# Nextomics/NextPolish2

Measured on AMD Instinct MI355X. Metric: polished reference Mbp/s (whole node) at 30x HiFi + k21/k31; FASTA identical to oracle, higher is better.
Workload: dtype u8

## Files before the change

### nextpolish2_amd/csrc/np2_ctx.hpp

```cpp
#pragma once
#include "../../include/np2.h"
#include "np2_abi.hpp"
#include "np2_common.hpp"
#include "np2_kernels.hpp"
#include "np2_hostcpu.hpp"

#include <algorithm>
#include <atomic>
#include <chrono>
#include <cstdio>
#include <cstdlib>
#include <cstring>
#include <map>
#include <memory>
#include <exception>
#include <mutex>
#include <stdexcept>
#include <string>
#include <vector>

namespace np2h {

using namespace np2;

// ... 488 lines not shown
    uint32_t chunk_epoch = 0;
    DevBuf<uint32_t> tile_cur, tile_n, tile_scan, tile_scanb, tile_nn, tile_nr, tile_noff, tile_roff;
    uint32_t tile_cap = TILE_CAP;
    uint32_t bucket_cap = 0;
    DevBuf<uint2> nrec;
    DevBuf<uint8_t> votebuf;
    DevBuf<uint32_t> band, band_n, band_off, row_cnt;
    DevBuf<int64_t> run_gain, tile_gain;
    DevBuf<uint8_t> out_snap;
    DevBuf<uint8_t> run_flag;
    uint32_t deep_min = 65536;
    DevBuf<uint32_t> lq_list, hbits;
    DevBuf<uint16_t> tile_pidx;
    bool pidx_valid = false;
    DevBuf<ReadInfo> rinfo;
    DevBuf<uint32_t> lqc, lqoff;
    DevBuf<uint8_t> pflag;
    DevBuf<uint32_t> dp_list;
    DevBuf<uint16_t> pf_slots;
    DevBuf<uint32_t> pf_bad, pf_bad2;
    DevBuf<uint64_t> pf_prof;
    bool front_fused = false;
    struct Hooks {
        bool front_unfused = false, pf_prof = false, edge_sort = false;
        bool test_misspeculate = false, shard_spec_log = false, phase_profile = false, exact_grow = false, no_speculate = false;
        bool has_grow_guess = false, rech_general = false, rech_log = false;
        uint32_t grow_guess = 0;
        uint32_t rech_cap_list = 0xFFFFFFFFu, rech_cap_jobs = 0xFFFFFFFFu, rech_cap_blob = 0xFFFFFFFFu;
        bool has_pf_cap = false, has_pf_cap_big = false, has_pf_halo = false, has_pf_cov_max = false;
        uint32_t pf_cap = 0, pf_cap_big = 0, pf_halo = 0, pf_cov_max = 0;
        void read() {
            auto on = [](const char *n) { return getenv(n) != nullptr; };
            auto u32 = [](const char *n, bool &has, uint32_t &v) {
                if (const char *e = getenv(n)) has = true, v = (uint32_t)atol(e);
            };
            front_unfused = on("NP2_FRONT_UNFUSED"), pf_prof = on("NP2_PF_PROF"), edge_sort = on("NP2_EDGE_SORT");
            test_misspeculate = on("NP2_TEST_MISSPECULATE");
            shard_spec_log = on("NP2_SHARD_SPEC_LOG"), phase_profile = on("NP2_PHASE_PROFILE"), exact_grow = on("NP2_EXACT_GROW");
            no_speculate = on("NP2_NO_SPECULATE");
            rech_general = on("NP2_RECH_GENERAL");
            rech_log = on("NP2_RECH_LOG");
            if (const char *e = getenv("NP2_TEST_RECH_CAP")) {
                char *end = nullptr;
                rech_cap_list = (uint32_t)strtoul(e, &end, 10);
                if (end && *end == ',') rech_cap_jobs = (uint32_t)strtoul(end + 1, &end, 10);
                if (end && *end == ',') rech_cap_blob = (uint32_t)strtoul(end + 1, &end, 10);
            }
            u32("NP2_TEST_GROW_GUESS", has_grow_guess, grow_guess);
            u32("NP2_PF_CAP", has_pf_cap, pf_cap), u32("NP2_PF_CAP_BIG", has_pf_cap_big, pf_cap_big);
            u32("NP2_PF_HALO", has_pf_halo, pf_halo), u32("NP2_PF_COV_MAX", has_pf_cov_max, pf_cov_max);
        }
    } hooks;
    bool pf_big = getenv("NP2_PF_BIG") != nullptr;
    uint32_t front_redos = 0;
    DevBuf<uint16_t> kscore_saved;
    DevBuf<uint8_t> sstr;
    DevBuf<uint64_t> soff;
    DevBuf<uint16_t> sscore;
};


namespace np2h {


enum Scal { S_ERR = 0, S_NNODES, S_NRUNS, S_BEST, S_PATHBEGIN, S_NRAW, S_NREG, S_DUP, S_LAST0, S_LAST1, S_GAIN0,
            S_GAIN1, S_DEEP, S_NDPLIST, S_NRECH, S_NGROUPS, S_NLONG, S_NLQ, S_PF, S_M0, S_M1, S_M2, S_M3, S_NC, S_SB, S_GROW,
            S_NBAD, S_PFOUT, S_PFGAIN0, S_PFGAIN1, S_PFEND0, S_PFEND1, S_NBAD2, S_NOKEY, S_COUNT = 34 };
static_assert(S_M1 % 2 == 0 && S_LAST0 % 2 == 0 && S_GAIN0 % 2 == 0 && S_PFGAIN0 % 2 == 0 && S_PFEND0 % 2 == 0,
              "64-bit device counters live in these slot pairs");

static constexpr int NP2_MAX_YAK = 15;
static constexpr uint32_t SCAL_TOTAL = 96;
static_assert(S_COUNT + 2 * (NP2_MAX_YAK + 2) <= SCAL_TOTAL && S_COUNT < 64, "round counters behind the posted block; the mailbox holds 64 words");
static constexpr uint32_t S_RL = S_COUNT + 2 * (NP2_MAX_YAK + 2);
static_assert(S_RL + 2 + np2::RL_STATE_WORDS <= SCAL_TOTAL, "the region lists' counters fit behind the round counters");

inline double thread_cpu_ms() {
    timespec ts;
    clock_gettime(CLOCK_THREAD_CPUTIME_ID, &ts);
    return ts.tv_sec * 1e3 + ts.tv_nsec * 1e-6;
}
struct WallTimer {
    np2_ctx *cx;
    const char *name;
    double t0, c0 = 0;
    WallTimer(np2_ctx *c, const char *n);
    ~WallTimer();
};

struct EventTimer {
// ... 245 lines not shown
```

### nextpolish2_amd/csrc/np2_host.cpp

```cpp
#include "../../include/np2.h"
#include "np2_common.hpp"
#include "np2_kernels.hpp"
#include "np2_ctx.hpp"
#include "np2_phase_host.hpp"

#include <algorithm>
#include <atomic>
#include <thread>
#include <chrono>
#include <cstdio>
#include <cstdlib>
#include <cstring>
#include <map>
#include <mutex>
#include <stdexcept>
#include <string>
#include <unordered_map>
#include <unordered_set>
#include <future>
#include <functional>
#include <vector>

using namespace np2;

// ... 100 lines not shown
    (void)cx;
    if (e & 4u) throw Np2Error(NP2_E_REFPANIC, "reference would panic: seq2 order is equal to 0");
    if (e & 8u) throw Np2Error(NP2_E_REFPANIC, "reference would panic: index out of bounds: lqseq.seqs[max1_p]");
    if (e & 16u) throw Np2Error(NP2_E_REFPANIC, "reference would panic: the first lqseq is not ref.");
    if (e & 32u) throw Np2Error(NP2_E_REFPANIC, "reference would panic: lqseq.seqs[0] after retain_sort_seqs");
    if (e & 64u) throw Np2Error(NP2_E_REFPANIC, "reference would panic: consensus index out of bounds in reupdate");
    if (e & 128u) throw Np2Error(NP2_E_NOMEM, "cartesian product of chained LQ regions is too large");
    if (e & LB_ERR) throw Np2Error(NP2_E_DEVICE, "device-wide scan timed out waiting for a predecessor block");
    if (e & (GROW_ERR | RECH_CAP_ERR)) throw GrowRetry((e & GROW_ERR) != 0, (e & RECH_CAP_ERR) != 0);
    if (e & LQ_LIST_ERR) throw Np2Error(NP2_E_DEVICE, "internal: more low-quality bases than their list was sized for");
}

struct VoteData {
    uint32_t R = 0;
    bool any = false;
    std::vector<uint64_t> pair_key;
    std::vector<uint32_t> pair_cnt;
    const uint64_t *view_key = nullptr;
    const uint32_t *view_cnt = nullptr;
    uint64_t view_n = 0;
    const uint32_t *off = nullptr;
    const phase::Graph::Edge *edges = nullptr;
    uint32_t n_nokey = 0;
    std::vector<uint32_t> off_own;
    std::vector<phase::Graph::Edge> edges_own;
    bool rows() const { return off != nullptr; }
    const uint64_t *keys() const { return view_key ? view_key : pair_key.data(); }
    const uint32_t *cnts() const { return view_key ? view_cnt : pair_cnt.data(); }
    uint64_t n_pairs() const { return view_key ? view_n : (uint64_t)pair_key.size(); }
    void own() {
        if (rows() && off_own.empty()) {
            off_own.assign(off, off + R + 1);
            edges_own.assign(edges, edges + off[R]);
            off = off_own.data(), edges = edges_own.data();
        }
        if (!view_key) return;
        pair_key.assign(view_key, view_key + view_n);
        pair_cnt.assign(view_cnt, view_cnt + view_n);
        view_key = nullptr, view_cnt = nullptr, view_n = 0;
    }
    std::vector<uint32_t> first_key;
    std::vector<int32_t> ref_w;
    std::vector<uint8_t> ref_seen, bad;
    const uint8_t *d_bad = nullptr;
    bool key_added = false;
};
// ... 50 lines not shown
        cx->ecount.ensure(n_reg + 2);
        cx->eoff.ensure(std::max<size_t>(n_reg + 2, (size_t)c->L + 2));
        const size_t RP = ((size_t)R + 63) & ~(size_t)63;
        const size_t band_words = (size_t)R * EDGE_BAND;
        const size_t b_v = RP * 10, b_off = (((size_t)R + 2) * 4 + 15) & ~(size_t)15;
        uint8_t *vbuf;
        uint32_t *row_off;
        if (wide) {
            cx->votebuf.ensure(b_v);
            cx->band_off.ensure((size_t)R + 2);
            vbuf = cx->votebuf.p, row_off = cx->band_off.p;
        } else {
            cx->votepack.ensure(b_v + b_off + band_words * 2 * sizeof(phase::Graph::Edge) + 64);
            vbuf = cx->votepack.p, row_off = (uint32_t *)(cx->votepack.p + b_v);
        }
        uint32_t *v_first = (uint32_t *)vbuf;
        int32_t *v_refw = (int32_t *)(vbuf + RP * 4);
        uint8_t *v_seen = vbuf + RP * 8, *v_bad = vbuf + RP * 9;
        op_fill(cx, v_first, 0xFF, RP * 4);
        op_fill(cx, v_refw, 0, RP * 6);
        launch_vote_phase(s, rt, asref, use_all, cx->lq_start.p, own_lo, own_hi, cx->reg_lable.p, cx->grp.p, cx->ecount.p,
                          v_refw, v_seen, v_bad, v_first, cx->scal.p + S_ERR);
        exclusive_total_n(cx, cx->ecount.p, cx->eoff.p, n_reg);
        launch_vote_counts(s, v_first, v_bad, R, cx->scal.p + S_M1);
        cx->band.ensure(band_words + 4);
        cx->band_n.ensure((size_t)R + 2);
        op_fill(cx, cx->scal.p + S_M3, 0, 4);
        launch_edges_row(s, rt, cx->grp.p, cx->ecount.p, cx->pj.p, cx->pcount.p, cx->alive.p, R, cx->band.p, cx->band_n.p,
                         cx->scal.p + S_M3);
        if (wide) {
            exclusive_total_n(cx, cx->band_n.p, row_off, R);
            cx->ekey.ensure(band_words + 2);
            cx->eval.ensure(band_words + 2);
            launch_band_emit(s, cx->band.p, R, row_off, cx->ekey.p, cx->eval.p, cx->scal.p + S_NRAW, key_add);
        } else {
            cx->row_cnt.ensure((size_t)R + 2);
            launch_vote_rows_count(s, cx->band.p, cx->band_n.p, v_bad, use_all, R, cx->row_cnt.p, cx->scal.p + S_NOKEY);
            exclusive_total_n(cx, cx->row_cnt.p, row_off, R);
            launch_vote_rows_emit(s, cx->band.p, cx->band_n.p, v_bad, use_all, v_first, R, row_off, cx->votepack.p + b_v + b_off,
                                  cx->scal.p + S_NRAW, cx->scal.p + S_NOKEY);
        }
    }
    const size_t RP = ((size_t)R + 63) & ~(size_t)63;
    const size_t b_v = RP * 10, b_off = (((size_t)R + 2) * 4 + 15) & ~(size_t)15;
    auto per_read = [&](const uint8_t *vb) {
        vd.first_key.assign((const uint32_t *)vb, (const uint32_t *)vb + R);
        vd.ref_w.assign((const int32_t *)(vb + RP * 4), (const int32_t *)(vb + RP * 4) + R);
        vd.ref_seen.assign(vb + RP * 8, vb + RP * 8 + R);
        vd.bad.assign(vb + RP * 9, vb + RP * 9 + R);
    };
    bool far = false, have_per_read = false;
    {
        std::vector<uint32_t> sc;
        uint8_t *pin = nullptr;
        const size_t EB = sizeof(phase::Graph::Edge);
        static_assert(sizeof(phase::Graph::Edge) == 8 && alignof(phase::Graph::Edge) <= 8, "an edge is {u32 neighbour, f32 weight}");
        const uint32_t likely = (uint32_t)std::min<size_t>((size_t)R * EDGE_BAND * 2, std::max<size_t>((size_t)R * 128, 1u << 15));
        if (wide) {
            sc = fetch_scal(cx, cx->scal.p + S_M0, cx->eoff.p + n_reg);
        } else {
            pin = (uint8_t *)cx->pin_d2h.ensure(b_v + b_off + (size_t)likely * EB + 64);
            const uint32_t seq = ++cx->mbox_seq;
            launch_post(cx->stream, cx->scal.p, S_COUNT, cx->mbox_dev, seq, cx->scal.p + S_M0, cx->eoff.p + n_reg, nullptr, nullptr,
                        nullptr, nullptr, nullptr, nullptr, nullptr, nullptr);
            op_d2h(cx, pin, cx->votepack.p, b_v + b_off);
            launch_copy_counted(cx->stream, (uint32_t *)(pin + b_v + b_off), (const uint32_t *)(cx->votepack.p + b_v + b_off),
                                (const uint32_t *)(cx->votepack.p + b_v) + R, likely * (uint32_t)(EB / 4), (uint32_t)(EB / 4));
            op_sync(cx);
            if (__atomic_load_n(&cx->mbox_host[0], __ATOMIC_ACQUIRE) != seq)
                throw Np2Error(NP2_E_DEVICE, "mailbox not posted after a synchronisation");
            sc.assign(cx->mbox_host + 1, cx->mbox_host + 1 + S_COUNT);
        }
        check_region_err(cx, sc[S_ERR]);
        pc.resolve(sc);
        NE = sc[S_M0];
        if (!cx->trace && sc[S_M1] == 0 && sc[S_M2] == 0) {
            if (NE) throw Np2Error(NP2_E_DEVICE, "internal: pair edges without voting reads");
            return;
        }
        NU = sc[S_NRAW];
        far = sc[S_M3] != 0 || cx->hooks.edge_sort;
        if (!wide) cx->timing.host.push_back({far ? "vote_sort" : "vote_rows", 1.0f});
        if (!wide) {
            per_read(pin);
            have_per_read = true;
            vd.d_bad = cx->votepack.p + RP * 9;
            if (!far) {
                if (NU > likely) {
                    pin = (uint8_t *)cx->pin_d2h.ensure(b_v + b_off + (size_t)NU * EB + 64);
                    op_d2h(cx, pin, cx->votepack.p, b_v + b_off + (size_t)NU * EB);
                    op_sync(cx);
                }
                vd.off = (const uint32_t *)(pin + b_v), vd.edges = (const phase::Graph::Edge *)(pin + b_v + b_off);
                vd.n_nokey = sc[S_NOKEY];
                if (vd.off[R] != NU) throw Np2Error(NP2_E_DEVICE, "internal: vote rows and edge count disagree");
            }
        }
    }
    vd.any = true;
    if (NE && far) {
        {
            EventTimer t(cx, "vote_phase");
            cx->ekey.ensure(NE + 2);
            cx->ekey_s.ensure(NE + 2);
            cx->eval.ensure(NE + 2);
// ... 29 lines not shown
            op_copy_d2d(cx, cx->votepack2.p + b_key, cx->eval.p, (size_t)NU * 4);
            if (b_pr) op_copy_d2d(cx, cx->votepack2.p + b_key + b_w, cx->votebuf.p, b_pr);
            op_d2h(cx, pin, cx->votepack2.p, b_key + b_w + b_pr);
        } else {
            op_d2h(cx, pin, cx->ekey.p, (size_t)NU * 8);
            op_d2h(cx, pin + b_key, cx->eval.p, (size_t)NU * 4);
            if (b_pr) op_d2h(cx, pin + b_key + b_w, cx->votebuf.p, b_pr);
        }
        op_sync(cx);
        vd.view_key = (const uint64_t *)pin, vd.view_cnt = (const uint32_t *)(pin + b_key), vd.view_n = NU;
        vd.key_added = wide && !far;
        if (b_pr) {
            per_read(pin + b_key + b_w);
            if (wide) vd.d_bad = cx->votebuf.p + RP * 9;
        }
    }
    if (cx->trace) {
        vd.own();
        trace_put(cx, pass, "hete.lable", d2h(cx, cx->reg_lable.p, n_reg));
        trace_put(cx, pass, "hete.kscore", d2h(cx, cx->kscore.p, pc.NC));
    }
}

std::vector<uint32_t> vote_decide(np2_ctx *cx, const VoteData &vd, bool use_all, int pass = -1) {
    if (!vd.any) return {};
    const uint32_t R = vd.R;
    const uint64_t NU = vd.rows() ? 0 : vd.n_pairs();
    const uint32_t *const pair_cnt = vd.rows() ? nullptr : vd.cnts();
    const double t_host0 = now_ms();
    std::vector<std::pair<uint32_t, uint32_t>> keys;
    for (uint32_t r = 0; r < R; ++r)
        if (vd.first_key[r] != 0xFFFFFFFFu) keys.emplace_back(vd.first_key[r], r);
    if (keys.size() < 4096) {
        std::sort(keys.begin(), keys.end());
    } else {
        std::vector<std::pair<uint32_t, uint32_t>> tmp(keys.size());
        std::vector<uint32_t> cnt(65537);
        for (int pass = 0; pass < 2; ++pass) {
            const int sh = 16 * pass;
            std::fill(cnt.begin(), cnt.end(), 0u);
            for (const auto &k : keys) ++cnt[((k.first >> sh) & 0xFFFFu) + 1];
            for (size_t i = 0; i < 65536; ++i) cnt[i + 1] += cnt[i];
            for (const auto &k : keys) tmp[cnt[(k.first >> sh) & 0xFFFFu]++] = k;
            keys.swap(tmp);
        }
    }
    const bool prof = getenv("NP2_PHASE_PROFILE") != nullptr;
    double t_mark = t_host0;
    auto mark = [&](const char *what) {
// ... 915 lines not shown
            if (cx->trace) trace_cns(cx, (int)r.pass, "cns_rech" + std::to_string(y), fetch_cns_dev(cx, cur));
        }
        fetch_result(cx, cur.pos, cur.base, cur.M_p, cur.M_cap, result, guessed ? r.M + r.grow_prev : r.M + pc.grow);
    } catch (const GrowRetry &g) {
        if ((g.grow && !guessed) || (g.rech_cap && !by_list)) throw;
        result.release();
        op_fill(cx, cx->scal.p + S_ERR, 0, 4);
        op_fill(cx, cx->scal.p + S_COUNT, 0, (size_t)(SCAL_TOTAL - S_COUNT) * 4);
        if (g.rech_cap) cx->timing.host.push_back({"rech_redo", 1.0f});
        r.reuse = false;
        run_final_pass(r, result, exact_grow || g.grow, rech_general || g.rech_cap);
    }
}

void polish_impl(np2_ctx *cx, np2_contig *c, const np2_opts_t *o, ResultOut &result) {
    PolishRun r;
    r.cx = cx, r.c = c, r.o = *o;
    run_begin(r);
    const bool no_spec = cx->hooks.no_speculate;
    const bool use_all = o->use_all_reads != 0;
    struct Decision {
        std::vector<uint32_t> losers;
        double ms = 0;
    };
    struct Pending {
        std::future<Decision> fut;
        std::shared_ptr<VoteData> vd;
        size_t n_bad = 0;
        bool active = false;
    } pend;
    auto settle = [&]() -> bool {
        if (!pend.active) return true;
        pend.active = false;
        Decision d = pend.fut.get();
        cx->timing.host.push_back({"wall_louvain", (float)d.ms});
        std::vector<uint32_t> extra;
        for (uint32_t id : d.losers) {
            REFPANIC_IF(id >= c->R, "index out of bounds: alignseqs[id]");
            if (!pend.vd->bad[id]) extra.push_back(id);
        }
        if (extra.empty() && d.losers.size() == pend.n_bad && !cx->hooks.test_misspeculate) return true;
        if (!extra.empty()) {
            cx->kill_ids.ensure(extra.size() + 1);
            h2d_staged(cx, cx->kill_ids.p, extra.data(), extra.size() * 4);
            launch_kill_reads(cx->stream, cx->kill_ids.p, (uint32_t)extra.size(), cx->alive.p);
        }
        r.reuse = false;
        r.front_issued = false;
        return false;
    };
    const std::function<void()> settle_then_redo = [&]() {
        if (!settle()) run_pass_front(r);
    };
    while (!r.final_pass()) {
        auto vd = std::make_shared<VoteData>();
        run_vote_pass(r, *vd, &settle_then_redo);
        size_t n_bad = 0;
        if (vd->any && vd->d_bad && !use_all && !cx->trace && !no_spec)
            for (uint8_t b : vd->bad) n_bad += b;
        if (n_bad == 0) {
            run_apply_losers(r, vote_decide(cx, *vd, use_all, (int)r.pass));
            continue;
        }
        launch_kill_flagged(cx->stream, vd->d_bad, c->R, cx->alive.p);
        ++r.pass;
        r.reuse = false;
        if (cx->hooks.pf_prof) vd->own();
        pass_front_issue(cx, c, r.T, (int)r.pass);
        r.front_issued = true;
        op_submit(cx);
        pend.vd = vd;
        pend.n_bad = n_bad;
        pend.active = true;
        auto decide = [vd, use_all]() {
            Decision d;
            const double t0 = now_ms();
            d.losers = vote_decide(nullptr, *vd, use_all);
            d.ms = now_ms() - t0;
            return d;
        };
        if (tl_recorder() == nullptr) {
            vd->own();
            pend.fut = std::async(std::launch::async, decide);
        } else {
            std::promise<Decision> p;
            pend.fut = p.get_future();
            try {
                p.set_value(decide());
            } catch (...) {
                p.set_exception(std::current_exception());
            }
            (void)settle();
        }
    }
    for (;;) {
        run_final_pass(r, result);
        if (settle()) break;
        result.release();
    }
}
// ... 811 lines not shown
            while (i < mk.size() && j < nx) {
                if (mk[i] < xk[j]) {
                    tk.push_back(mk[i]), tc.push_back(mc[i]), ++i;
                } else if (xk[j] < mk[i]) {
                    tk.push_back(xk[j]), tc.push_back(xc[j]), ++j;
                } else {
                    const uint32_t same = (mc[i] & 0xFFFFu) + (xc[j] & 0xFFFFu), neg = (mc[i] >> 16) + (xc[j] >> 16);
                    if (same > 0xFFFFu || neg > 0xFFFFu) return NP2_E_UNSUPPORTED;
                    tk.push_back(mk[i]), tc.push_back(same | (neg << 16)), ++i, ++j;
                }
            }
            tk.insert(tk.end(), mk.begin() + (long)i, mk.end());
            tc.insert(tc.end(), mc.begin() + (long)i, mc.end());
            tk.insert(tk.end(), xk + j, xk + nx);
            tc.insert(tc.end(), xc + j, xc + nx);
            mk.swap(tk), mc.swap(tc);
        }
        if (!vd.view_key) {
            vd.pair_key.swap(mk);
            vd.pair_cnt.swap(mc);
        }
        for (uint32_t r = 0; r < n_reads_total; ++r)
            if (votes_any[r]) vd.first_key[r] = 0xFFFFFFFEu - first_pos[r];
        if (getenv("NP2_VOTE_COMPACT")) {
            if (!vote_rows_from_pairs(vd, opts->use_all_reads != 0)) return NP2_E_UNSUPPORTED;
        }
        std::vector<uint32_t> ls = vote_decide(nullptr, vd, opts->use_all_reads != 0);
        *n_losers = (uint32_t)ls.size();
        for (size_t i = 0; i < ls.size(); ++i) losers[i] = ls[i];
        return NP2_OK;
    });
}

int np2_shard_apply(np2_shard_run_t *h, const uint32_t *losers, uint32_t n) {
    ShardRun *sr = (ShardRun *)h;
    if (!sr || (n && !losers) || (sr->run.final_pass() && !sr->spec)) return NP2_E_ARG;
    np2_ctx *cx = sr->run.cx;
    return abi_guard([&] {
        std::vector<uint32_t> local;
        const np2_shard_plan_t &pl = sr->plan;
        for (uint32_t i = 0; i < n; ++i) {
            if (losers[i] == 0) throw Np2Error(NP2_E_REFPANIC, "reference would panic: the contig itself was voted out");
            if (losers[i] >= pl.read_lo && losers[i] < pl.read_hi) local.push_back(losers[i] - pl.read_lo + 1);
        }
        if (sr->spec) {
            sr->spec = false;
            std::vector<uint32_t> extra, spared;
            size_t n_flagged = 0;
// ... 156 lines not shown
```

### nextpolish2_amd/csrc/np2_kernels.hpp

```cpp
#pragma once
#include <cstddef>
#include <cstdint>
#include <hip/hip_runtime.h>
#include "../../include/np2.h"
#include "np2_lookback.hpp"
#include "np2_launch.hpp"

namespace np2 {

static constexpr uint32_t TILE_SHIFT = 10;
static constexpr uint32_t TILE = 1u << TILE_SHIFT;
static constexpr uint32_t TILE_CAP = 4096;

static constexpr uint32_t DENSE_COLS = 4096;
struct ChunkDesc {
    uint64_t nib_off;
    uint64_t ckbase;
    uint32_t read, ts;
    uint32_t c0, ncols;
    uint32_t first_chunk;
    uint32_t aln_t_e, nck;
    uint32_t pad0;
    uint32_t pad[4];
};
// ... 238 lines not shown

struct RegionTables {
    const uint32_t *cand_off;
    const uint32_t *order;
    uint16_t *kscore;
    const uint32_t *seq_off;
    const uint8_t *seq;
    uint32_t n_reg;
};
struct RechPtrs {
    const void *groups;
    const uint32_t *job_off;
    const uint32_t *rech;
    const uint32_t *cand_off;
    const uint32_t *keep_list;
    const uint32_t *seq_off;
    const uint8_t *seq;
    const uint8_t *cns_base;
    uint32_t n_groups;
};
void launch_vote_phase(hipStream_t s, const RegionTables &rt, bool asref, bool use_all, const uint32_t *lq_start,
                       uint32_t own_lo, uint32_t own_hi, uint8_t *reg_lable, uint8_t *grp, uint32_t *ecount, int32_t *ref_w,
                       uint8_t *ref_seen, uint8_t *bad, uint32_t *first_reg, uint32_t *err);
void launch_vote_counts(hipStream_t s, const uint32_t *first_reg, const uint8_t *bad, uint32_t R, uint32_t *out);
void launch_edges_write(hipStream_t s, const RegionTables &rt, const uint8_t *reg_lable, const uint8_t *grp,
                        const uint32_t *ecount, const uint32_t *eoff, uint64_t *ekey, uint32_t *eval);
static constexpr uint32_t EDGE_BAND = 256;
void launch_edges_row(hipStream_t s, const RegionTables &rt, const uint8_t *grp, const uint32_t *ecount, const uint32_t *pj,
                      const uint32_t *pcount, const uint8_t *alive, uint32_t R, uint32_t *band, uint32_t *row_n, uint32_t *ovf);
void launch_band_emit(hipStream_t s, const uint32_t *band, uint32_t R, const uint32_t *row_off, uint64_t *ukey, uint32_t *uw,
                      uint32_t *n_out, uint64_t key_add = 0);
void launch_vote_rows_count(hipStream_t s, const uint32_t *band, const uint32_t *row_n, const uint8_t *bad, bool use_all, uint32_t R,
                            uint32_t *cnt, uint32_t *nokey);
void launch_vote_rows_emit(hipStream_t s, const uint32_t *band, const uint32_t *row_n, const uint8_t *bad, bool use_all,
                           const uint32_t *first_reg, uint32_t R, const uint32_t *off, void *edges, uint32_t *n_out, uint32_t *nokey);
void launch_edge_reduce(hipStream_t s, const uint64_t *ekey, const uint32_t *eval, uint32_t n, uint32_t *flag, uint32_t *wout);
void launch_edge_compact(hipStream_t s, const uint64_t *ekey, const uint32_t *flag, const uint32_t *idx, const uint32_t *wout,
                         uint32_t n, uint64_t *ukey, uint32_t *uw, uint32_t *n_out);
void launch_seed(hipStream_t s, const RegionTables &rt, int32_t max_indel_len, uint8_t *reg_lable, uint32_t *seed_cand,
                 uint32_t *keep_n, uint32_t *keep_list, uint16_t *keep_ks, uint32_t *err, uint32_t *rl_list = nullptr,
                 uint32_t *rl_cnt = nullptr, uint32_t rl_cap = 0);
uint32_t region_lb_blocks(uint32_t n_reg);
void launch_splice_find(hipStream_t s, const uint32_t *cns_pos, const uint32_t *M_p, const uint32_t *lq_start,
                        const uint32_t *lq_end, const uint8_t *reg_lable, uint8_t lable, uint32_t n_reg, uint32_t *idx_s,
                        uint32_t *idx_e, uint32_t *stuck);
void launch_splice_plan(hipStream_t s, const Lookback &lb, const uint8_t *reg_lable, uint8_t lable, uint32_t n_reg,
                        const uint32_t *stuck, const uint32_t *idx_s, const uint32_t *idx_e, const uint32_t *seed_cand,
                        const uint32_t *seq_off, uint32_t *ap_g, uint32_t *ap_s, uint32_t *ap_e, int32_t *ap_delta,
                        int32_t *ap_shift_incl, uint32_t *n_ap, const uint32_t *M_in, uint32_t *M_out, uint32_t out_cap , uint32_t *err);
void launch_splice_write(hipStream_t s, const uint32_t *in_pos, const uint8_t *in_base, const uint32_t *M_p, uint32_t M_cap,
                         const uint32_t *ap_g, const uint32_t *ap_s, const uint32_t *ap_e, const int32_t *ap_delta,
                         const int32_t *ap_shift_incl, const uint32_t *n_ap, uint32_t max_ap, const uint32_t *lq_start,
                         const uint32_t *seed_cand, const uint32_t *seq_off, const uint8_t *seq, uint32_t *out_pos,
                         uint8_t *out_base);
void launch_shard_bounds(hipStream_t s, const uint32_t *cns_pos, const uint32_t *M_p, const uint32_t *t, uint32_t *out);
void launch_rech_list(hipStream_t s, const Lookback &lb, const uint8_t *reg_lable, uint32_t n_reg, uint32_t *rech,
                      uint32_t *n_rech, unsigned long long *blob_bound, uint32_t *err);
void launch_rech_groups(hipStream_t s, const Lookback &lb, const uint32_t *rech, const uint32_t *n_rech_p, uint32_t max_rech,
// ... 71 lines not shown
```

### nextpolish2_amd/csrc/np2_regions.hip

```cpp
#include "np2_common.hpp"
#include "np2_kernels.hpp"
#include "np2_blockscan.hpp"
#include "np2_lookback.hpp"

namespace np2 {

static constexpr uint8_t LB_TEMP = 0x01, LB_SUCC = 0x80, LB_HETE = 0x40, LB_RECH = 0x20;

__device__ __forceinline__ uint32_t min_support(uint32_t n) { return n >= 9 ? 3u : (n >= 6 ? 2u : 1u); }

struct SubWave {
    uint32_t base;
    bool half;
    __device__ __forceinline__ uint64_t ballot(bool p) const {
        const uint64_t b = __ballot(p);
        return half ? (b >> base) & 0xFFFFFFFFull : b;
    }
    template <class T> __device__ __forceinline__ T shfl(T v, uint32_t j) const { return __shfl(v, (int)(base + j)); }
};

struct WaveStats {
    uint64_t eqmask;
    uint32_t stat;
    uint32_t c;
// ... 221 lines not shown
        gi = grp[c0 + lane];
        v = rt.kscore[c0 + lane] > 0;
    }
    uint64_t V = __ballot(v);
    if ((V & 1ull) && __shfl(order, 0) == 0) V &= ~1ull;
    const bool mine = (V >> lane) & 1ull;
    const uint32_t cnt = mine ? __builtin_popcountll(lane == 63 ? 0ull : (V >> (lane + 1))) : 0u;
    uint32_t inc = cnt;
    for (int o = 1; o < 64; o <<= 1) {
        const uint32_t t = __shfl_up(inc, o);
        if (lane >= (uint32_t)o) inc += t;
    }
    uint32_t o = eoff[g] + inc - cnt;
    for (uint32_t j = 1; j < n; ++j) {
        const uint32_t oj = __shfl(order, j), gj = __shfl(gi, j);
        if (mine && j > lane && ((V >> j) & 1ull)) {
            ekey[o] = ((uint64_t)order << 32) | oj;
            eval[o] = (gj == gi) ? 1u : 0xFFFFFFFFu;
            ++o;
        }
    }
}

__device__ __forceinline__ void k_edges_row(const uint32_t np2_bid0, const uint32_t np2_nb, RegionTables rt, const uint8_t *__restrict__ grp,
                                            const uint32_t *__restrict__ ecount, const uint32_t *__restrict__ pj,
                                            const uint32_t *__restrict__ pcount, const uint8_t *__restrict__ alive, uint32_t R,
                                            uint32_t *__restrict__ band, uint32_t *__restrict__ row_n, uint32_t *__restrict__ ovf) {
    const uint32_t np2_bid = xcd_order(np2_bid0, np2_nb);
    __shared__ uint32_t s_row[4][EDGE_BAND];
    const uint32_t lane = threadIdx.x & 63, wv = (uint32_t)__builtin_amdgcn_readfirstlane((int)(threadIdx.x >> 6));
    const uint32_t a = np2_bid * 4 + wv;
    if (a >= R) return;
    uint32_t *row = s_row[wv];
    *reinterpret_cast<uint4 *>(row + lane * 4) = make_uint4(0, 0, 0, 0);
    uint32_t far = 0;
    const uint32_t n_span = (a != 0 && alive[a]) ? pcount[a] : 0u;
    const uint32_t j0 = n_span ? pj[a] : 0u;
    const uint32_t hl = lane & 31, hsel = lane >> 5;
    for (uint32_t base = 0; base < n_span; base += 64) {
        const uint32_t gl = j0 + base + lane;
        const bool in = base + lane < n_span && gl < rt.n_reg;
        const uint32_t c0l = in ? rt.cand_off[gl] : 0u, c1l = in ? rt.cand_off[gl + 1] : 0u;
        uint64_t het = __ballot(in && ecount[gl] != 0);
        while (het) {
            const uint32_t i0 = (uint32_t)__builtin_ctzll(het);
            het &= het - 1;
            const uint32_t c0a = (uint32_t)__builtin_amdgcn_readlane((int)c0l, (int)i0);
            const uint32_t na = (uint32_t)__builtin_amdgcn_readlane((int)c1l, (int)i0) - c0a;
            uint32_t c0b = 0, nb = 0;
            bool two = false;
// ... 17 lines not shown
            if ((V & 1ull) && __shfl(order, 0) == 0) V &= ~1ull;
            if (two && ((V >> 32) & 1ull) && __shfl(order, 32) == 0) V &= ~(1ull << 32);
            const uint64_t me = __ballot(order == a) & V;
            const uint64_t half_mask = two ? (hsel ? 0xFFFFFFFF00000000ull : 0x00000000FFFFFFFFull) : ~0ull;
            const uint64_t mine = me & half_mask;
            if (!me) continue;
            const uint32_t ga = __shfl(gi, mine ? (int)__builtin_ctzll(mine) : 0);
            if (mine && ((V >> lane) & 1ull) && order > a) {
                const uint32_t d = order - a - 1;
                if (d < EDGE_BAND)
                    atomicAdd(&row[d], gi == ga ? 1u : 0x10000u);
                else
                    ++far;
            }
        }
    }
    const uint4 w = *reinterpret_cast<const uint4 *>(row + lane * 4);
    uint32_t c = (w.x != 0) + (w.y != 0) + (w.z != 0) + (w.w != 0);
    for (int o = 32; o > 0; o >>= 1) c += __shfl_xor(c, o);
    if (c) *reinterpret_cast<uint4 *>(band + (uint64_t)a * EDGE_BAND + lane * 4) = w;
    if (lane == 0) row_n[a] = c;
    for (int o = 32; o > 0; o >>= 1) far += __shfl_xor(far, o);
    if (far && lane == 0) atomicAdd(ovf, far);
}
__device__ __forceinline__ void k_band_emit(const uint32_t np2_bid, const uint32_t np2_nb, const uint32_t *__restrict__ band, uint32_t R,
                                            const uint32_t *__restrict__ row_off, uint64_t *__restrict__ ukey,
                                            uint32_t *__restrict__ ucnt, uint32_t *__restrict__ n_out, uint64_t key_add) {
    const uint32_t lane = threadIdx.x & 63;
    const uint32_t a = (uint32_t)__builtin_amdgcn_readfirstlane((int)((np2_bid * blockDim.x + threadIdx.x) >> 6));
    if (a >= R) return;
    if (a == R - 1 && lane == 0) *n_out = row_off[R];
    if (row_off[a + 1] == row_off[a]) return;
    const uint4 w = *reinterpret_cast<const uint4 *>(band + (uint64_t)a * EDGE_BAND + lane * 4);
    const uint32_t v[4] = {w.x, w.y, w.z, w.w};
    const uint32_t c = (w.x != 0) + (w.y != 0) + (w.z != 0) + (w.w != 0);
    uint32_t inc = c;
    for (int o = 1; o < 64; o <<= 1) {
        const uint32_t t = __shfl_up(inc, o);
        if (lane >= (uint32_t)o) inc += t;
    }
    uint32_t o = row_off[a] + inc - c;
#pragma unroll
    for (uint32_t k = 0; k < 4; ++k)
        if (v[k]) {
            ukey[o] = (((uint64_t)a << 32) | (a + 1 + lane * 4 + k)) + key_add;
            ucnt[o] = v[k];
            ++o;
        }
}

__device__ __forceinline__ uint32_t vote_row_above(const uint32_t *__restrict__ band, const uint8_t *__restrict__ bad, uint32_t use_all,
                                                   uint32_t R, uint32_t v, uint32_t d) {
    const uint32_t b = v + 1 + d;
    if (b >= R) return 0;
    const uint32_t w = band[(uint64_t)v * EDGE_BAND + d];
    return (w != 0 && (use_all || !bad[b])) ? w : 0u;
}
__device__ __forceinline__ uint32_t vote_row_below(const uint32_t *__restrict__ band, const uint32_t *__restrict__ row_n,
                                                   const uint8_t *__restrict__ bad, uint32_t use_all, uint32_t v, int64_t a) {
    if (a < 1 || a >= (int64_t)v || v - (uint32_t)a > EDGE_BAND) return 0;
    if (row_n[a] == 0 || (!use_all && bad[a])) return 0;
    return band[(uint64_t)a * EDGE_BAND + (v - (uint32_t)a - 1)];
}
__device__ __forceinline__ float vote_weight(uint32_t w) {
    const int32_t same = (int32_t)(w & 0xFFFFu), neg = (int32_t)(w >> 16);
    return (float)(neg >= 3 ? -neg : same - neg);
}
__device__ __forceinline__ void k_vote_rows_count(const uint32_t np2_bid, const uint32_t np2_nb, const uint32_t *__restrict__ band,
                                                  const uint32_t *__restrict__ row_n, const uint8_t *__restrict__ bad, uint32_t use_all,
                                                  uint32_t R, uint32_t *__restrict__ cnt, uint32_t *__restrict__ nokey) {
    const uint32_t lane = threadIdx.x & 63;
    const uint32_t v = (uint32_t)__builtin_amdgcn_readfirstlane((int)((np2_bid * blockDim.x + threadIdx.x) >> 6));
    if (v >= R) return;
    if (v == 0 && lane == 0) *nokey = 0;
    uint32_t c = 0;
    if (v != 0 && (use_all || !bad[v])) {
        const bool own = row_n[v] != 0;
#pragma unroll
        for (uint32_t k = 0; k < EDGE_BAND / 64; ++k) {
            const uint32_t d = k * 64 + lane;
            if (own) c += vote_row_above(band, bad, use_all, R, v, d) != 0;
            c += vote_row_below(band, row_n, bad, use_all, v, (int64_t)v - 1 - d) != 0;
        }
    }
    for (int o = 32; o > 0; o >>= 1) c += __shfl_xor(c, o);
    if (lane == 0) cnt[v] = c;
}
__device__ __forceinline__ void k_vote_rows_emit(const uint32_t np2_bid, const uint32_t np2_nb, const uint32_t *__restrict__ band,
                                                 const uint32_t *__restrict__ row_n, const uint8_t *__restrict__ bad, uint32_t use_all,
                                                 const uint32_t *__restrict__ first_reg, uint32_t R, const uint32_t *__restrict__ off,
                                                 uint2 *__restrict__ edges, uint32_t *__restrict__ n_out, uint32_t *__restrict__ nokey) {
    const uint32_t lane = threadIdx.x & 63;
    const uint32_t v = (uint32_t)__builtin_amdgcn_readfirstlane((int)((np2_bid * blockDim.x + threadIdx.x) >> 6));
    if (v >= R) return;
    if (v == R - 1 && lane == 0) *n_out = off[R];
    if (v == 0) return;
    const bool own = row_n[v] != 0, live = use_all || !bad[v];
    const uint64_t lt = (1ull << lane) - 1;
    uint32_t o = off[v];
    const uint32_t end = off[v + 1];
    if (live && end != o) {
#pragma unroll
        for (uint32_t k = 0; k < EDGE_BAND / 64; ++k) {
            const int64_t a = (int64_t)v - EDGE_BAND + k * 64 + lane;
            const uint32_t w = vote_row_below(band, row_n, bad, use_all, v, a);
            const uint64_t m = __ballot(w != 0);
            const uint32_t at = o + (uint32_t)__popcll(m & lt);
            if (w != 0 && at < end) edges[at] = make_uint2((uint32_t)a, __float_as_uint(vote_weight(w)));
            o += (uint32_t)__popcll(m);
        }
    }
    if (!own) return;
    const bool v_key = first_reg[v] != 0xFFFFFFFFu;
    uint32_t nk = 0;
#pragma unroll
    for (uint32_t k = 0; k < EDGE_BAND / 64; ++k) {
        const uint32_t d = k * 64 + lane, b = v + 1 + d;
        if (b < R && band[(uint64_t)v * EDGE_BAND + d] != 0 && !(v_key && first_reg[b] != 0xFFFFFFFFu)) ++nk;
        const uint32_t w = live ? vote_row_above(band, bad, use_all, R, v, d) : 0u;
// ... 851 lines not shown
    if (tid == 0) splice_plan_total(M, dsum, cnt, out_cap, n_ap, M_out, err);
    uint32_t keep[RL_ITEMS], ksum = 0;
#pragma unroll
    for (uint32_t k = 0; k < RL_ITEMS; ++k) {
        keep[k] = 0;
        if (tid * RL_ITEMS + k < n) {
            const uint8_t l = rech_relabel(reg_lable[g[k]]);
            reg_lable[g[k]] = l;
            keep[k] = (l & LB_RECH) ? 1u : 0u;
        }
        ksum += keep[k];
    }
    uint32_t n_keep;
    uint32_t lk = block_excl_scan<OpAdd, 4>(ksum, sh, n_keep);
#pragma unroll
    for (uint32_t k = 0; k < RL_ITEMS; ++k) {
        if (keep[k]) a.list_out[lk] = g[k];
        lk += keep[k];
    }
    if (tid == 0) *a.cnt_in = 0, *a.cnt_out = last_round ? 0u : n_keep;
}

__device__ __forceinline__ void k_vote_counts(const uint32_t np2_bid, const uint32_t np2_nb, const uint32_t *__restrict__ first_reg, const uint8_t *__restrict__ bad,
                                                      uint32_t R, uint32_t *__restrict__ out) {
    __shared__ uint32_t sk[16], sb[16];
    uint32_t nk = 0, nb = 0;
    for (uint32_t r = threadIdx.x; r < R; r += 1024) {
        nk += first_reg[r] != 0xFFFFFFFFu ? 1u : 0u;
        nb += bad[r] ? 1u : 0u;
    }
    for (int o = 32; o > 0; o >>= 1) {
        nk += __shfl_xor(nk, o);
        nb += __shfl_xor(nb, o);
    }
    if ((threadIdx.x & 63) == 0) {
        sk[threadIdx.x >> 6] = nk;
        sb[threadIdx.x >> 6] = nb;
    }
    __syncthreads();
    if (threadIdx.x == 0) {
        uint32_t a = 0, b = 0;
        for (int i = 0; i < 16; ++i) {
            a += sk[i];
            b += sb[i];
        }
        out[0] = a;
        out[1] = b;
    }
}

static inline dim3 g1(uint64_t n, uint32_t bs = 256) { return dim3((unsigned)((n + bs - 1) / bs)); }

void launch_vote_phase(hipStream_t s, const RegionTables &rt, bool asref, bool use_all, const uint32_t *lq_start,
                       uint32_t own_lo, uint32_t own_hi, uint8_t *reg_lable, uint8_t *grp, uint32_t *ecount, int32_t *ref_w,
                       uint8_t *ref_seen, uint8_t *bad, uint32_t *first_reg, uint32_t *err) {
    if (rt.n_reg)
        NP2_LAUNCH(k_vote_phase, g1((uint64_t)((rt.n_reg + 1) / 2) * 64), 256, s, rt, asref ? 1u : 0u, use_all ? 1u : 0u, lq_start, own_lo, own_hi, reg_lable, grp, ecount, ref_w, ref_seen, bad, first_reg, err);
}
void launch_vote_counts(hipStream_t s, const uint32_t *first_reg, const uint8_t *bad, uint32_t R, uint32_t *out) {
    NP2_LAUNCH(k_vote_counts, dim3(1), 1024, s, first_reg, bad, R, out);
}
void launch_edges_write(hipStream_t s, const RegionTables &rt, const uint8_t *reg_lable, const uint8_t *grp,
                        const uint32_t *ecount, const uint32_t *eoff, uint64_t *ekey, uint32_t *eval) {
    if (rt.n_reg)
        NP2_LAUNCH(k_edges_write, g1((uint64_t)rt.n_reg * 64), 256, s, rt, reg_lable, grp, ecount, eoff, ekey, eval);
}
void launch_edges_row(hipStream_t s, const RegionTables &rt, const uint8_t *grp, const uint32_t *ecount, const uint32_t *pj,
                      const uint32_t *pcount, const uint8_t *alive, uint32_t R, uint32_t *band, uint32_t *row_n, uint32_t *ovf) {
    if (R) NP2_LAUNCH(k_edges_row, g1((uint64_t)R * 64), 256, s, rt, grp, ecount, pj, pcount, alive, R, band, row_n, ovf);
}
void launch_vote_rows_count(hipStream_t s, const uint32_t *band, const uint32_t *row_n, const uint8_t *bad, bool use_all, uint32_t R,
                            uint32_t *cnt, uint32_t *nokey) {
    if (R) NP2_LAUNCH(k_vote_rows_count, g1((uint64_t)R * 64), 256, s, band, row_n, bad, use_all ? 1u : 0u, R, cnt, nokey);
}
void launch_vote_rows_emit(hipStream_t s, const uint32_t *band, const uint32_t *row_n, const uint8_t *bad, bool use_all,
                           const uint32_t *first_reg, uint32_t R, const uint32_t *off, void *edges, uint32_t *n_out, uint32_t *nokey) {
    if (R) NP2_LAUNCH(k_vote_rows_emit, g1((uint64_t)R * 64), 256, s, band, row_n, bad, use_all ? 1u : 0u, first_reg, R, off, (uint2 *)edges, n_out, nokey);
}
void launch_band_emit(hipStream_t s, const uint32_t *band, uint32_t R, const uint32_t *row_off, uint64_t *ukey, uint32_t *uw,
                      uint32_t *n_out, uint64_t key_add) {
    if (R) NP2_LAUNCH(k_band_emit, g1((uint64_t)R * 64), 256, s, band, R, row_off, ukey, uw, n_out, key_add);
}
void launch_edge_reduce(hipStream_t s, const uint64_t *ekey, const uint32_t *eval, uint32_t n, uint32_t *flag,
                        uint32_t *wout) {
    if (n) NP2_LAUNCH(k_edge_reduce, g1(n), 256, s, ekey, eval, n, flag, wout);
}
void launch_edge_compact(hipStream_t s, const uint64_t *ekey, const uint32_t *flag, const uint32_t *idx,
                         const uint32_t *wout, uint32_t n, uint64_t *ukey, uint32_t *uw, uint32_t *n_out) {
    if (n) NP2_LAUNCH(k_edge_compact, g1(n), 256, s, ekey, flag, idx, wout, n, ukey, uw, n_out);
}
void launch_seed(hipStream_t s, const RegionTables &rt, int32_t max_indel_len, uint8_t *reg_lable, uint32_t *seed_cand,
                 uint32_t *keep_n, uint32_t *keep_list, uint16_t *keep_ks, uint32_t *err, uint32_t *rl_list, uint32_t *rl_cnt,
                 uint32_t rl_cap) {
    if (rt.n_reg)
        NP2_LAUNCH(k_seed, g1((uint64_t)((rt.n_reg + 1) / 2) * 64), 256, s, rt, max_indel_len, reg_lable, seed_cand, keep_n, keep_list, keep_ks, err, rl_list, rl_cnt, rl_cap);
}
uint32_t region_lb_blocks(uint32_t n_reg) { return (n_reg + 256 * LB_REG_ITEMS - 1) / (256 * LB_REG_ITEMS); }
void launch_splice_find(hipStream_t s, const uint32_t *cns_pos, const uint32_t *M_p, const uint32_t *lq_start,
                        const uint32_t *lq_end, const uint8_t *reg_lable, uint8_t lable, uint32_t n_reg,
                        uint32_t *idx_s, uint32_t *idx_e, uint32_t *stuck) {
// ... 79 lines not shown
```

Measured before the change: 4488.

## Skip vote Louvain clustering when no negative-weight read pairs exist

Counts negative-weight live read pairs on the device inside the edge-row kernel. When that count is zero, the row count and emit kernels skip their work and the host decision returns the bad reads directly instead of running Louvain community detection. A parallel host scan does the same check for the pair-key path. The shortcut assumes that with no negative edges the clustering always flags only the bad reads. If that assumption is wrong in an edge case, output could differ, and the new atomic counter adds a little work to every edge-row launch.

```diff
diff --git a/nextpolish2_amd/csrc/np2_ctx.hpp b/nextpolish2_amd/csrc/np2_ctx.hpp
--- a/nextpolish2_amd/csrc/np2_ctx.hpp
+++ b/nextpolish2_amd/csrc/np2_ctx.hpp
@@ -534,7 +534,7 @@
     DevBuf<uint64_t> pf_prof;
     bool front_fused = false;
     struct Hooks {
-        bool front_unfused = false, pf_prof = false, edge_sort = false;
+        bool front_unfused = false, pf_prof = false, edge_sort = false, vote_no_skip = false;
         bool test_misspeculate = false, shard_spec_log = false, phase_profile = false, exact_grow = false, no_speculate = false;
         bool has_grow_guess = false, rech_general = false, rech_log = false;
         uint32_t grow_guess = 0;
@@ -550,6 +550,7 @@
             test_misspeculate = on("NP2_TEST_MISSPECULATE");
             shard_spec_log = on("NP2_SHARD_SPEC_LOG"), phase_profile = on("NP2_PHASE_PROFILE"), exact_grow = on("NP2_EXACT_GROW");
             no_speculate = on("NP2_NO_SPECULATE");
+            vote_no_skip = on("NP2_VOTE_NO_SKIP");
             rech_general = on("NP2_RECH_GENERAL");
             rech_log = on("NP2_RECH_LOG");
             if (const char *e = getenv("NP2_TEST_RECH_CAP")) {
@@ -577,7 +578,7 @@
 
 enum Scal { S_ERR = 0, S_NNODES, S_NRUNS, S_BEST, S_PATHBEGIN, S_NRAW, S_NREG, S_DUP, S_LAST0, S_LAST1, S_GAIN0,
             S_GAIN1, S_DEEP, S_NDPLIST, S_NRECH, S_NGROUPS, S_NLONG, S_NLQ, S_PF, S_M0, S_M1, S_M2, S_M3, S_NC, S_SB, S_GROW,
-            S_NBAD, S_PFOUT, S_PFGAIN0, S_PFGAIN1, S_PFEND0, S_PFEND1, S_NBAD2, S_NOKEY, S_COUNT = 34 };
+            S_NBAD, S_PFOUT, S_PFGAIN0, S_PFGAIN1, S_PFEND0, S_PFEND1, S_NBAD2, S_NOKEY, S_VNEG, S_COUNT = 35 };
 static_assert(S_M1 % 2 == 0 && S_LAST0 % 2 == 0 && S_GAIN0 % 2 == 0 && S_PFGAIN0 % 2 == 0 && S_PFEND0 % 2 == 0,
               "64-bit device counters live in these slot pairs");
 
diff --git a/nextpolish2_amd/csrc/np2_host.cpp b/nextpolish2_amd/csrc/np2_host.cpp
--- a/nextpolish2_amd/csrc/np2_host.cpp
+++ b/nextpolish2_amd/csrc/np2_host.cpp
@@ -146,6 +146,8 @@
     const uint32_t *off = nullptr;
     const phase::Graph::Edge *edges = nullptr;
     uint32_t n_nokey = 0;
+    bool neg_valid = false, no_skip = false;
+    uint32_t n_neg = 0;
     std::vector<uint32_t> off_own;
     std::vector<phase::Graph::Edge> edges_own;
     bool rows() const { return off != nullptr; }
@@ -242,23 +244,25 @@
         launch_vote_phase(s, rt, asref, use_all, cx->lq_start.p, own_lo, own_hi, cx->reg_lable.p, cx->grp.p, cx->ecount.p,
                           v_refw, v_seen, v_bad, v_first, cx->scal.p + S_ERR);
         exclusive_total_n(cx, cx->ecount.p, cx->eoff.p, n_reg);
-        launch_vote_counts(s, v_first, v_bad, R, cx->scal.p + S_M1);
+        launch_vote_counts(s, v_first, v_bad, R, cx->scal.p + S_M1, cx->scal.p + S_VNEG);
         cx->band.ensure(band_words + 4);
         cx->band_n.ensure((size_t)R + 2);
         op_fill(cx, cx->scal.p + S_M3, 0, 4);
         launch_edges_row(s, rt, cx->grp.p, cx->ecount.p, cx->pj.p, cx->pcount.p, cx->alive.p, R, cx->band.p, cx->band_n.p,
-                         cx->scal.p + S_M3);
+                         cx->scal.p + S_M3, v_bad, use_all, cx->scal.p + S_VNEG);
         if (wide) {
             exclusive_total_n(cx, cx->band_n.p, row_off, R);
             cx->ekey.ensure(band_words + 2);
             cx->eval.ensure(band_words + 2);
             launch_band_emit(s, cx->band.p, R, row_off, cx->ekey.p, cx->eval.p, cx->scal.p + S_NRAW, key_add);
         } else {
+            const bool may_skip = !cx->trace && !cx->hooks.vote_no_skip;
             cx->row_cnt.ensure((size_t)R + 2);
-            launch_vote_rows_count(s, cx->band.p, cx->band_n.p, v_bad, use_all, R, cx->row_cnt.p, cx->scal.p + S_NOKEY);
+            launch_vote_rows_count(s, cx->band.p, cx->band_n.p, v_bad, use_all, R, cx->row_cnt.p, cx->scal.p + S_NOKEY,
+                                   cx->scal.p + S_VNEG, may_skip);
             exclusive_total_n(cx, cx->row_cnt.p, row_off, R);
             launch_vote_rows_emit(s, cx->band.p, cx->band_n.p, v_bad, use_all, v_first, R, row_off, cx->votepack.p + b_v + b_off,
-                                  cx->scal.p + S_NRAW, cx->scal.p + S_NOKEY);
+                                  cx->scal.p + S_NRAW, cx->scal.p + S_NOKEY, cx->scal.p + S_VNEG, may_skip);
         }
     }
     const size_t RP = ((size_t)R + 63) & ~(size_t)63;
@@ -301,6 +305,11 @@
         NU = sc[S_NRAW];
         far = sc[S_M3] != 0 || cx->hooks.edge_sort;
         if (!wide) cx->timing.host.push_back({far ? "vote_sort" : "vote_rows", 1.0f});
+        vd.no_skip = cx->hooks.vote_no_skip || cx->trace;
+        if (!wide && !far) {
+            vd.neg_valid = true, vd.n_neg = sc[S_VNEG];
+            cx->timing.host.push_back({"vote_neg", (float)vd.n_neg});
+        }
         if (!wide) {
             per_read(pin);
             have_per_read = true;
@@ -376,9 +385,44 @@
     }
 }
 
-std::vector<uint32_t> vote_decide(np2_ctx *cx, const VoteData &vd, bool use_all, int pass = -1) {
+static bool vote_has_no_negative(const VoteData &vd, bool use_all) {
+    if (vd.rows()) return vd.neg_valid && vd.n_neg == 0;
+    const uint64_t *k = vd.keys();
+    const uint32_t *cn = vd.cnts();
+    const uint32_t R = vd.R;
+    const uint8_t *skip = use_all ? nullptr : vd.bad.data();
+    std::vector<uint8_t> found(phase::host_threads(), 0);
+    phase::parallel_ranges((size_t)vd.n_pairs(), (size_t)1 << 18, [&](unsigned t, size_t lo, size_t hi) {
+        for (size_t i = lo; i < hi; ++i) {
+            const uint32_t a = (uint32_t)(k[i] >> 32), b = (uint32_t)k[i];
+            if (a >= R || b >= R || vd.first_key[a] == 0xFFFFFFFFu || vd.first_key[b] == 0xFFFFFFFFu) {
+                found[t] = 1;
+                return;
+            }
+            if (skip && (skip[a] | skip[b])) continue;
+            const int32_t same = (int32_t)(cn[i] & 0xFFFFu), neg = (int32_t)(cn[i] >> 16);
+            if ((neg >= 3 ? -neg : same - neg) < 0) {
+                found[t] = 1;
+                return;
+            }
+        }
+    });
+    for (uint8_t f : found)
+        if (f) return false;
+    return true;
+}
+std::vector<uint32_t> vote_decide(np2_ctx *cx, const VoteData &vd, bool use_all, int pass = -1, bool *skipped = nullptr) {
+    if (skipped) *skipped = false;
     if (!vd.any) return {};
     const uint32_t R = vd.R;
+    if (!vd.no_skip && vote_has_no_negative(vd, use_all)) {
+        if (cx) cx->timing.host.push_back({"vote_skip", 1.0f});
+        if (skipped) *skipped = true;
+        std::vector<uint32_t> flagged;
+        for (uint32_t r = 0; r < R; ++r)
+            if (vd.bad[r]) flagged.push_back(r);
+        return flagged;
+    }
     const uint64_t NU = vd.rows() ? 0 : vd.n_pairs();
     const uint32_t *const pair_cnt = vd.rows() ? nullptr : vd.cnts();
     const double t_host0 = now_ms();
@@ -1340,6 +1384,7 @@
     struct Decision {
         std::vector<uint32_t> losers;
         double ms = 0;
+        bool skipped = false;
     };
     struct Pending {
         std::future<Decision> fut;
@@ -1351,7 +1396,8 @@
         if (!pend.active) return true;
         pend.active = false;
         Decision d = pend.fut.get();
-        cx->timing.host.push_back({"wall_louvain", (float)d.ms});
+        if (d.skipped) cx->timing.host.push_back({"vote_skip", 1.0f});
+        else cx->timing.host.push_back({"wall_louvain", (float)d.ms});
         std::vector<uint32_t> extra;
         for (uint32_t id : d.losers) {
             REFPANIC_IF(id >= c->R, "index out of bounds: alignseqs[id]");
@@ -1393,7 +1439,7 @@
         auto decide = [vd, use_all]() {
             Decision d;
             const double t0 = now_ms();
-            d.losers = vote_decide(nullptr, *vd, use_all);
+            d.losers = vote_decide(nullptr, *vd, use_all, -1, &d.skipped);
             d.ms = now_ms() - t0;
             return d;
         };
@@ -2251,8 +2297,10 @@
         }
         for (uint32_t r = 0; r < n_reads_total; ++r)
             if (votes_any[r]) vd.first_key[r] = 0xFFFFFFFEu - first_pos[r];
+        vd.no_skip = getenv("NP2_VOTE_NO_SKIP") != nullptr;
         if (getenv("NP2_VOTE_COMPACT")) {
             if (!vote_rows_from_pairs(vd, opts->use_all_reads != 0)) return NP2_E_UNSUPPORTED;
+            vd.no_skip = true;
         }
         std::vector<uint32_t> ls = vote_decide(nullptr, vd, opts->use_all_reads != 0);
         *n_losers = (uint32_t)ls.size();
diff --git a/nextpolish2_amd/csrc/np2_kernels.hpp b/nextpolish2_amd/csrc/np2_kernels.hpp
--- a/nextpolish2_amd/csrc/np2_kernels.hpp
+++ b/nextpolish2_amd/csrc/np2_kernels.hpp
@@ -284,18 +284,20 @@
 void launch_vote_phase(hipStream_t s, const RegionTables &rt, bool asref, bool use_all, const uint32_t *lq_start,
                        uint32_t own_lo, uint32_t own_hi, uint8_t *reg_lable, uint8_t *grp, uint32_t *ecount, int32_t *ref_w,
                        uint8_t *ref_seen, uint8_t *bad, uint32_t *first_reg, uint32_t *err);
-void launch_vote_counts(hipStream_t s, const uint32_t *first_reg, const uint8_t *bad, uint32_t R, uint32_t *out);
+void launch_vote_counts(hipStream_t s, const uint32_t *first_reg, const uint8_t *bad, uint32_t R, uint32_t *out, uint32_t *neg_pairs);
 void launch_edges_write(hipStream_t s, const RegionTables &rt, const uint8_t *reg_lable, const uint8_t *grp,
                         const uint32_t *ecount, const uint32_t *eoff, uint64_t *ekey, uint32_t *eval);
 static constexpr uint32_t EDGE_BAND = 256;
 void launch_edges_row(hipStream_t s, const RegionTables &rt, const uint8_t *grp, const uint32_t *ecount, const uint32_t *pj,
-                      const uint32_t *pcount, const uint8_t *alive, uint32_t R, uint32_t *band, uint32_t *row_n, uint32_t *ovf);
+                      const uint32_t *pcount, const uint8_t *alive, uint32_t R, uint32_t *band, uint32_t *row_n, uint32_t *ovf,
+                      const uint8_t *bad, bool use_all, uint32_t *neg_pairs);
 void launch_band_emit(hipStream_t s, const uint32_t *band, uint32_t R, const uint32_t *row_off, uint64_t *ukey, uint32_t *uw,
                       uint32_t *n_out, uint64_t key_add = 0);
 void launch_vote_rows_count(hipStream_t s, const uint32_t *band, const uint32_t *row_n, const uint8_t *bad, bool use_all, uint32_t R,
-                            uint32_t *cnt, uint32_t *nokey);
+                            uint32_t *cnt, uint32_t *nokey, const uint32_t *neg_pairs, bool may_skip);
 void launch_vote_rows_emit(hipStream_t s, const uint32_t *band, const uint32_t *row_n, const uint8_t *bad, bool use_all,
-                           const uint32_t *first_reg, uint32_t R, const uint32_t *off, void *edges, uint32_t *n_out, uint32_t *nokey);
+                           const uint32_t *first_reg, uint32_t R, const uint32_t *off, void *edges, uint32_t *n_out, uint32_t *nokey,
+                           const uint32_t *neg_pairs, bool may_skip);
 void launch_edge_reduce(hipStream_t s, const uint64_t *ekey, const uint32_t *eval, uint32_t n, uint32_t *flag, uint32_t *wout);
 void launch_edge_compact(hipStream_t s, const uint64_t *ekey, const uint32_t *flag, const uint32_t *idx, const uint32_t *wout,
                          uint32_t n, uint64_t *ukey, uint32_t *uw, uint32_t *n_out);
diff --git a/nextpolish2_amd/csrc/np2_regions.hip b/nextpolish2_amd/csrc/np2_regions.hip
--- a/nextpolish2_amd/csrc/np2_regions.hip
+++ b/nextpolish2_amd/csrc/np2_regions.hip
@@ -267,10 +267,15 @@
     }
 }
 
+__device__ __forceinline__ float vote_weight(uint32_t w) {
+    const int32_t same = (int32_t)(w & 0xFFFFu), neg = (int32_t)(w >> 16);
+    return (float)(neg >= 3 ? -neg : same - neg);
+}
 __device__ __forceinline__ void k_edges_row(const uint32_t np2_bid0, const uint32_t np2_nb, RegionTables rt, const uint8_t *__restrict__ grp,
                                             const uint32_t *__restrict__ ecount, const uint32_t *__restrict__ pj,
                                             const uint32_t *__restrict__ pcount, const uint8_t *__restrict__ alive, uint32_t R,
-                                            uint32_t *__restrict__ band, uint32_t *__restrict__ row_n, uint32_t *__restrict__ ovf) {
+                                            uint32_t *__restrict__ band, uint32_t *__restrict__ row_n, uint32_t *__restrict__ ovf,
+                                            const uint8_t *__restrict__ bad, uint32_t use_all, uint32_t *__restrict__ neg_pairs) {
     const uint32_t np2_bid = xcd_order(np2_bid0, np2_nb);
     __shared__ uint32_t s_row[4][EDGE_BAND];
     const uint32_t lane = threadIdx.x & 63, wv = (uint32_t)__builtin_amdgcn_readfirstlane((int)(threadIdx.x >> 6));
@@ -334,6 +339,17 @@
     if (lane == 0) row_n[a] = c;
     for (int o = 32; o > 0; o >>= 1) far += __shfl_xor(far, o);
     if (far && lane == 0) atomicAdd(ovf, far);
+    uint32_t ng = 0;
+    if (c && (use_all || !bad[a])) {
+        const uint32_t wk[4] = {w.x, w.y, w.z, w.w};
+#pragma unroll
+        for (uint32_t k = 0; k < 4; ++k) {
+            const uint32_t b = a + 1 + lane * 4 + k;
+            if (wk[k] != 0 && b < R && vote_weight(wk[k]) < 0.f && (use_all || !bad[b])) ++ng;
+        }
+        for (int o = 32; o > 0; o >>= 1) ng += __shfl_xor(ng, o);
+    }
+    if (ng && lane == 0) atomicAdd(neg_pairs, ng);
 }
 __device__ __forceinline__ void k_band_emit(const uint32_t np2_bid, const uint32_t np2_nb, const uint32_t *__restrict__ band, uint32_t R,
                                             const uint32_t *__restrict__ row_off, uint64_t *__restrict__ ukey,
@@ -374,19 +390,17 @@
     if (row_n[a] == 0 || (!use_all && bad[a])) return 0;
     return band[(uint64_t)a * EDGE_BAND + (v - (uint32_t)a - 1)];
 }
-__device__ __forceinline__ float vote_weight(uint32_t w) {
-    const int32_t same = (int32_t)(w & 0xFFFFu), neg = (int32_t)(w >> 16);
-    return (float)(neg >= 3 ? -neg : same - neg);
-}
 __device__ __forceinline__ void k_vote_rows_count(const uint32_t np2_bid, const uint32_t np2_nb, const uint32_t *__restrict__ band,
                                                   const uint32_t *__restrict__ row_n, const uint8_t *__restrict__ bad, uint32_t use_all,
-                                                  uint32_t R, uint32_t *__restrict__ cnt, uint32_t *__restrict__ nokey) {
+                                                  uint32_t R, uint32_t *__restrict__ cnt, uint32_t *__restrict__ nokey,
+                                                  const uint32_t *__restrict__ neg_pairs, uint32_t may_skip) {
     const uint32_t lane = threadIdx.x & 63;
     const uint32_t v = (uint32_t)__builtin_amdgcn_readfirstlane((int)((np2_bid * blockDim.x + threadIdx.x) >> 6));
     if (v >= R) return;
     if (v == 0 && lane == 0) *nokey = 0;
+    const bool skip = may_skip && *neg_pairs == 0;
     uint32_t c = 0;
-    if (v != 0 && (use_all || !bad[v])) {
+    if (!skip && v != 0 && (use_all || !bad[v])) {
         const bool own = row_n[v] != 0;
 #pragma unroll
         for (uint32_t k = 0; k < EDGE_BAND / 64; ++k) {
@@ -401,12 +415,13 @@
 __device__ __forceinline__ void k_vote_rows_emit(const uint32_t np2_bid, const uint32_t np2_nb, const uint32_t *__restrict__ band,
                                                  const uint32_t *__restrict__ row_n, const uint8_t *__restrict__ bad, uint32_t use_all,
                                                  const uint32_t *__restrict__ first_reg, uint32_t R, const uint32_t *__restrict__ off,
-                                                 uint2 *__restrict__ edges, uint32_t *__restrict__ n_out, uint32_t *__restrict__ nokey) {
+                                                 uint2 *__restrict__ edges, uint32_t *__restrict__ n_out, uint32_t *__restrict__ nokey,
+                                                 const uint32_t *__restrict__ neg_pairs, uint32_t may_skip) {
     const uint32_t lane = threadIdx.x & 63;
     const uint32_t v = (uint32_t)__builtin_amdgcn_readfirstlane((int)((np2_bid * blockDim.x + threadIdx.x) >> 6));
     if (v >= R) return;
     if (v == R - 1 && lane == 0) *n_out = off[R];
-    if (v == 0) return;
+    if (v == 0 || (may_skip && *neg_pairs == 0)) return;
     const bool own = row_n[v] != 0, live = use_all || !bad[v];
     const uint64_t lt = (1ull << lane) - 1;
     uint32_t o = off[v];
@@ -1304,8 +1319,9 @@
 }
 
 __device__ __forceinline__ void k_vote_counts(const uint32_t np2_bid, const uint32_t np2_nb, const uint32_t *__restrict__ first_reg, const uint8_t *__restrict__ bad,
-                                                      uint32_t R, uint32_t *__restrict__ out) {
+                                                      uint32_t R, uint32_t *__restrict__ out, uint32_t *__restrict__ neg_pairs) {
     __shared__ uint32_t sk[16], sb[16];
+    if (threadIdx.x == 0) *neg_pairs = 0;
     uint32_t nk = 0, nb = 0;
     for (uint32_t r = threadIdx.x; r < R; r += 1024) {
         nk += first_reg[r] != 0xFFFFFFFFu ? 1u : 0u;
@@ -1339,8 +1355,8 @@
     if (rt.n_reg)
         NP2_LAUNCH(k_vote_phase, g1((uint64_t)((rt.n_reg + 1) / 2) * 64), 256, s, rt, asref ? 1u : 0u, use_all ? 1u : 0u, lq_start, own_lo, own_hi, reg_lable, grp, ecount, ref_w, ref_seen, bad, first_reg, err);
 }
-void launch_vote_counts(hipStream_t s, const uint32_t *first_reg, const uint8_t *bad, uint32_t R, uint32_t *out) {
-    NP2_LAUNCH(k_vote_counts, dim3(1), 1024, s, first_reg, bad, R, out);
+void launch_vote_counts(hipStream_t s, const uint32_t *first_reg, const uint8_t *bad, uint32_t R, uint32_t *out, uint32_t *neg_pairs) {
+    NP2_LAUNCH(k_vote_counts, dim3(1), 1024, s, first_reg, bad, R, out, neg_pairs);
 }
 void launch_edges_write(hipStream_t s, const RegionTables &rt, const uint8_t *reg_lable, const uint8_t *grp,
                         const uint32_t *ecount, const uint32_t *eoff, uint64_t *ekey, uint32_t *eval) {
@@ -1348,16 +1364,18 @@
         NP2_LAUNCH(k_edges_write, g1((uint64_t)rt.n_reg * 64), 256, s, rt, reg_lable, grp, ecount, eoff, ekey, eval);
 }
 void launch_edges_row(hipStream_t s, const RegionTables &rt, const uint8_t *grp, const uint32_t *ecount, const uint32_t *pj,
-                      const uint32_t *pcount, const uint8_t *alive, uint32_t R, uint32_t *band, uint32_t *row_n, uint32_t *ovf) {
-    if (R) NP2_LAUNCH(k_edges_row, g1((uint64_t)R * 64), 256, s, rt, grp, ecount, pj, pcount, alive, R, band, row_n, ovf);
+                      const uint32_t *pcount, const uint8_t *alive, uint32_t R, uint32_t *band, uint32_t *row_n, uint32_t *ovf,
+                      const uint8_t *bad, bool use_all, uint32_t *neg_pairs) {
+    if (R) NP2_LAUNCH(k_edges_row, g1((uint64_t)R * 64), 256, s, rt, grp, ecount, pj, pcount, alive, R, band, row_n, ovf, bad, use_all ? 1u : 0u, neg_pairs);
 }
 void launch_vote_rows_count(hipStream_t s, const uint32_t *band, const uint32_t *row_n, const uint8_t *bad, bool use_all, uint32_t R,
-                            uint32_t *cnt, uint32_t *nokey) {
-    if (R) NP2_LAUNCH(k_vote_rows_count, g1((uint64_t)R * 64), 256, s, band, row_n, bad, use_all ? 1u : 0u, R, cnt, nokey);
+                            uint32_t *cnt, uint32_t *nokey, const uint32_t *neg_pairs, bool may_skip) {
+    if (R) NP2_LAUNCH(k_vote_rows_count, g1((uint64_t)R * 64), 256, s, band, row_n, bad, use_all ? 1u : 0u, R, cnt, nokey, neg_pairs, may_skip ? 1u : 0u);
 }
 void launch_vote_rows_emit(hipStream_t s, const uint32_t *band, const uint32_t *row_n, const uint8_t *bad, bool use_all,
-                           const uint32_t *first_reg, uint32_t R, const uint32_t *off, void *edges, uint32_t *n_out, uint32_t *nokey) {
-    if (R) NP2_LAUNCH(k_vote_rows_emit, g1((uint64_t)R * 64), 256, s, band, row_n, bad, use_all ? 1u : 0u, first_reg, R, off, (uint2 *)edges, n_out, nokey);
+                           const uint32_t *first_reg, uint32_t R, const uint32_t *off, void *edges, uint32_t *n_out, uint32_t *nokey,
+                           const uint32_t *neg_pairs, bool may_skip) {
+    if (R) NP2_LAUNCH(k_vote_rows_emit, g1((uint64_t)R * 64), 256, s, band, row_n, bad, use_all ? 1u : 0u, first_reg, R, off, (uint2 *)edges, n_out, nokey, neg_pairs, may_skip ? 1u : 0u);
 }
 void launch_band_emit(hipStream_t s, const uint32_t *band, uint32_t R, const uint32_t *row_off, uint64_t *ukey, uint32_t *uw,
                       uint32_t *n_out, uint64_t key_add) {
```

Result: faster. 4574, median of 6 (+1.9%).
